# belinghy/SteppingStone

Measured on AMD Instinct MI355X. Metric: env-steps/sec (batched random-action rollout), higher is better.
Workload: dtype f32; 1 GPU; Walker3DStepperEnv-v0, 4096 envs per MI355X, curriculum 0 (flat terrain), on-device Philox U(-1,1) actions, auto-reset on; envs_total=4096, parallelism=env-shard x1, ranks=1, steps_per_launch=1000, prewarm_steps=256

## Files before the change

steppingstone_amd/csrc/ss_dynamics.hpp:

```cpp
#pragma once
#include "ss_math.hpp"
#include "ss_pair.hpp"

namespace ss {

constexpr float kH = 1.0f / 240.0f;
constexpr float kDt = 1.0f / 60.0f;
constexpr float kGrav = 9.8f;
constexpr float kPlankA = kStonePlankHalfLength, kPlankB = kStonePlankHalfWidth;
constexpr int kPgsIters = 5;
constexpr float kErp = 0.2f;
constexpr float kSlop = 0.001f;
constexpr float kVcorrMax = 2.0f;


constexpr int kWave = 64;
constexpr int kEnvsPerWave = 32;
constexpr int kLdsSlots = 40;
constexpr int kSlotsA = 20;
constexpr int kLdsC = 0;
constexpr int kLdsT = 18;
constexpr int kLdsHead = 36;
constexpr int kScalarBase = kSlotsA * kWave * 4;
constexpr int kRecWords = 9;
constexpr int kCholWords = 15 + 6;
constexpr int kHandJc = 0, kHandL0 = kHandJc + 8 * kRecWords, kHandLc = kHandL0 + kCholWords, kHandDet = 129, kHandAct = 146, kHandFloats = 158, kHandCs = kHandLc;
constexpr bool bias_offload(int helpers) { return helpers >= 3; }
constexpr bool spine_packed(int helpers) { return helpers >= 3; }
constexpr bool torques_paired(int helpers, bool kstep) { return helpers >= 3 && kstep; }
constexpr bool response_from_lds(int helpers, bool kstep) { return helpers >= 3 && kstep; }
constexpr int kHandBias = kHandJc;
static_assert(24 <= 3 * kRecWords, "biases fit the spine records' place");
constexpr int kHandRows = kHandJc + 3 * kRecWords;
constexpr int kHandRows3 = 160;
constexpr int kHandFloats3 = kHandRows3 + 40;
constexpr int kHandSlots3 = (kHandFloats3 + 3) / 4;
constexpr int hand_slots(int helpers) { return helpers >= 3 ? kHandSlots3 : (kHandFloats + 3) / 4; }
constexpr bool rows_offload(int helpers) { return helpers >= 3; }
constexpr int kHandSlots = (kHandFloats + 3) / 4;
static_assert(kLdsSlots + kHandSlots <= 80, "two helper-variant workgroups must fit the 160 KiB of a CU (16384 envs: 512 workgroups)");
static_assert(kHandRows + 40 <= kHandJc + 8 * kRecWords, "rows fit the leg records' place");
constexpr int kHandBase = kLdsSlots * kWave * 4;
constexpr int kFarWord0 = kHandLc;
constexpr int kFarBytes = (kHandBase + kFarWord0 * kWave) * 4;
static_assert(kFarBytes <= 65536, "every hand-off word beyond the offset field of the lane's own base goes through the far base");
constexpr bool hand_far(int idx) { return idx >= kFarWord0; }
constexpr int hand_far_offset(int idx) { return (idx - kFarWord0) * kWave * 4; }
constexpr int lds_bytes(int helpers) { return (kLdsSlots + hand_slots(helpers)) * kWave * 16; }
constexpr int hand_last_word(int helpers) { return hand_slots(helpers) * 4 - 1; }
static_assert(kHandFloats3 - 1 <= hand_last_word(3) && kHandFloats + 2 - 1 <= hand_last_word(1), "the words in use (one helper: + kHandOut2's two) are allocated");
static_assert(kFarBytes + (kWave - 1) * 4 + hand_far_offset(hand_last_word(1)) + 4 <= lds_bytes(1), "one helper: far base + largest word is inside the allocation");
static_assert(kFarBytes + (kWave - 1) * 4 + hand_far_offset(hand_last_word(3)) + 4 <= lds_bytes(3), "three helpers: far base + largest word is inside the allocation");
static_assert(hand_far_offset(kFarWord0) == 0 && hand_far_offset(hand_last_word(3)) < 65536 && hand_far_offset(hand_last_word(1)) < 65536,
              "every far offset fits the 16-bit offset field");
static_assert(hand_far_offset(1) - hand_far_offset(0) == 256 && hand_far_offset(hand_last_word(3)) / 256 <= 255,
              "far offsets are multiples of 256 B within ds_*2st64_b32's reach");
constexpr int NH = 12;
enum { S_ACT = 0, S_Q = 12, S_QD = 24, S_WLAM = 36, S_POS = 48, S_QUAT = 51, S_VW = 55, S_VV = 58, S_STP = 61, S_STN = 70,
       S_WKEY = 79, S_END = 80 };
static_assert(S_END <= (kLdsSlots - kSlotsA) * 4, "LDS scalar region overflow");
constexpr bool warm_in_lds(int helpers) { return helpers < 3; }
constexpr bool reset_pose_offload(int helpers, bool kstep) { return helpers >= 3 && kstep; }
constexpr int S_POSE = S_WLAM;
static_assert(!(reset_pose_offload(0, true) && warm_in_lds(0)) && !(reset_pose_offload(1, true) && warm_in_lds(1)) &&
              !(reset_pose_offload(2, true) && warm_in_lds(2)) && !(reset_pose_offload(3, true) && warm_in_lds(3)),
              "the reset pose lives where the warm-start impulses would: only a kernel that keeps those in registers has the words to spare");
static_assert(S_POSE + NH <= S_POS, "twelve words");
#ifndef SS_ARM_TAIL
#define SS_ARM_TAIL 1
#endif
#ifndef SS_BASE_TAIL
#define SS_BASE_TAIL 1
#endif
constexpr bool arm_tail_offload(int helpers, bool kstep) { return SS_ARM_TAIL != 0 && helpers >= 3 && kstep; }
constexpr bool base_tail_offload(int helpers, bool kstep) { return SS_BASE_TAIL != 0 && helpers >= 3 && kstep; }
constexpr bool limb_tail_offload(int helpers, bool kstep) { return arm_tail_offload(helpers, kstep) || base_tail_offload(helpers, kstep); }
constexpr int kHandArm = kHandRows3, kHandDv0 = kHandDet, kHandV0f = kHandDv0 + 6;
constexpr int kArmHelper = 1, kBaseHelper = 2;
static_assert(kHandArm + 4 * kRecWords <= kHandRows3 + 36, "the arm records fit the rows' directions");
static_assert(kHandV0f + 6 <= kHandDet + 13, "dv0 and v0f stay below the detection's flags word and the sole");
#ifndef SS_SPINE_TAU
#define SS_SPINE_TAU 1
#endif
constexpr bool spine_tau_offload(int helpers, bool kstep) { return SS_SPINE_TAU != 0 && helpers >= 3 && kstep; }
constexpr int kHandTau = kHandCs + 2 * NH, kTauHelper = 1;
static_assert(kHandTau >= kHandCs + 2 * NH && kHandTau + 6 <= kHandLc + 36 && kHandLc + 36 <= kHandDet,
              "the spine torques lie behind cos / sin, inside Lambda_own's 36 words, below the detection's");
static_assert(hand_far(kHandTau) && hand_far_offset(kHandTau + 5) <= hand_far_offset(hand_last_word(3)), "far words inside the three-helper allocation");
static_assert(bias_offload(3) && kTauHelper == 1, "the spine torques ride on helper 1's bias job");

constexpr int kHalf[NH] = {0, 1, 2, 3, 4, 5, 6, 7, 13, 14, 15, 16};
constexpr int left_twin(int jr) { return jr < 3 ? jr : (jr < 8 ? jr + 5 : jr + 4); }
constexpr bool mirror_flips(int j) { return kAxis[j] != 1; }
__host__ __device__ constexpr float mirror_sign(int j, float m) { return mirror_flips(j) ? m : 1.f; }
__host__ __device__ constexpr float action_lane_sign(int jr, float m) {
  return jr < 3 ? mirror_sign(jr, m) : (float)kPolicySign[jr];
}
__host__ __device__ constexpr float policy_true_sign(int jr, int side) {
  return jr < 3 ? 1.f : (float)kPolicySign[jr] * ((mirror_flips(jr) && side) ? -1.f : 1.f);
}
constexpr int first_child_half(int b) {
  int r = -1;
  for (int i = 0; i < NH; ++i)
    if (kParent[kHalf[i]] == b) r = kHalf[i] + 1;
  return r;
}

#define SS_MEMBAR() asm volatile("" ::: "memory")
#if defined(__HIP_DEVICE_COMPILE__)
#define SS_WAVE_SYNC() asm volatile("" ::: "memory")
#else
#define SS_WAVE_SYNC() ss_host_wave_sync()
#endif

#if defined(SS_PROFILE_PHASES) && defined(__HIP_DEVICE_COMPILE__)
struct Prof { uint32_t t[16]; uint32_t last; };
#define SS_PROF_DECL Prof& prof,
#define SS_PROF_ARG prof,
#define SS_PROF_RAW(i) do { uint32_t _n = __builtin_amdgcn_readfirstlane((uint32_t)__builtin_amdgcn_s_memtime()); \
    prof.t[i] = __builtin_amdgcn_readfirstlane(prof.t[i] + (_n - __builtin_amdgcn_readfirstlane(prof.last))); prof.last = _n; } while (0)
#ifdef SS_PROFILE_EPILOGUE
#define SS_PROF(i) SS_PROF_RAW(0)
#define SS_PROFE(i) SS_PROF_RAW(i)
#else
#define SS_PROF(i) SS_PROF_RAW(i)
#define SS_PROFE(i) ((void)0)
#endif
#else
#define SS_PROFE(i) ((void)0)
struct Prof { int unused; };
#define SS_PROF_DECL
#define SS_PROF_ARG
#define SS_PROF(i) ((void)0)
#endif

#if defined(SS_FUZZ_SCHED) && defined(__HIP_DEVICE_COMPILE__)
__device__ __forceinline__ void ss_fuzz(uint32_t site) {
  uint32_t h = (uint32_t)__builtin_amdgcn_s_memtime() ^ (site * 0x9E3779B9u);
  h *= 0x85EBCA6Bu; h ^= h >> 13; h *= 0xC2B2AE35u; h ^= h >> 16;
  h = __builtin_amdgcn_readfirstlane(h);
  const uint32_t n = ((h >> 8) & 3u) == 0u ? (h & 255u) : (h & 15u);
#pragma unroll 1
  for (uint32_t i = 0; i < n; ++i) __builtin_amdgcn_s_sleep(1);
}
#define SS_FUZZ(site) ss_fuzz(site)
#else
#define SS_FUZZ(site) ((void)0)
#endif

constexpr bool cs_offload(int helpers) { return helpers >= 3; }

struct Lds {
  float* base;
  int lane;
  SSD float2& q2(int item) const { return reinterpret_cast<float2*>(base)[item * kWave + lane]; }
  SSD float& s(int idx) const { return base[kScalarBase + idx * kWave + lane]; }
  SSD float& hs(int idx) const {
#if defined(__HIP_DEVICE_COMPILE__)
    if (hand_far(idx)) {
      int off = kFarBytes + lane * 4;
      asm("" : "+v"(off));
      return *reinterpret_cast<float*>(reinterpret_cast<char*>(base) + off + hand_far_offset(idx));
    }
#endif
    return base[kHandBase + idx * kWave + lane];
  }
};

struct Stones {
  float p[3][3], nrm[3][3], tilt[3][2];
};

struct FootReport {
  int contact;
  int on_target;
  float sole[3];
};

struct Warm {
  float lam[4][3];
  int key;
};
SSD void warm_clear(Warm& w) {
#pragma unroll
  for (int k = 0; k < 4; ++k) w.lam[k][0] = w.lam[k][1] = w.lam[k][2] = 0.f;
  w.key = 0;
}

template <class T>
struct JRecT {
  T cs, sn, Uw[3], Uv[3], Dinv, u;
};
using JRec = JRecT<float>;
using JRec2 = JRecT<ssf2>;
static_assert(sizeof(JRec2) == 2 * sizeof(JRec), "a pair record is two scalar records, nothing else");
struct JointCache {
  JRec r[NH];
  Chol6 L0;
};
constexpr int half_pos(int j) { return j <= 7 ? j : j - 5; }
SSD void put_rec_at(const Lds& L, int w, const JRec& r) {
  L.hs(w + 0) = r.cs; L.hs(w + 1) = r.sn; L.hs(w + 2) = r.Dinv;
#pragma unroll
  for (int m = 0; m < 3; ++m) { L.hs(w + 3 + m) = r.Uw[m]; L.hs(w + 6 + m) = r.Uv[m]; }
}
SSD void get_rec_at(const Lds& L, int w, JRec& r) {
  r.cs = L.hs(w + 0); r.sn = L.hs(w + 1); r.Dinv = L.hs(w + 2);
#pragma unroll
  for (int m = 0; m < 3; ++m) { r.Uw[m] = L.hs(w + 3 + m); r.Uv[m] = L.hs(w + 6 + m); }
}
SSD void put_rec(const Lds& L, int k, const JRec& r) { put_rec_at(L, kHandJc + k * kRecWords, r); }
SSD void get_rec(const Lds& L, int k, JRec& r) { get_rec_at(L, kHandJc + k * kRecWords, r); }
SSD void put_chol(const Lds& L, const Chol6& c) {
#pragma unroll
  for (int m = 0; m < 15; ++m) L.hs(kHandL0 + m) = c.l[m];
#pragma unroll
  for (int m = 0; m < 6; ++m) L.hs(kHandL0 + 15 + m) = c.di[m];
}
SSD void get_chol(const Lds& L, Chol6& c) {
#pragma unroll
  for (int i = 0; i < 15; ++i) c.l[i] = L.hs(kHandL0 + i);
#pragma unroll
  for (int i = 0; i < 6; ++i) c.di[i] = L.hs(kHandL0 + 15 + i);
}

SSD float xchg(float x) {
#if defined(__HIP_DEVICE_COMPILE__)
  return __builtin_bit_cast(float, __builtin_amdgcn_mov_dpp(__builtin_bit_cast(int, x), 0xB1, 0xF, 0xF, true));
#else
  return ss_host_xchg(x);
#endif
}
SSD uint32_t xchg_u32(uint32_t x) {
#if defined(__HIP_DEVICE_COMPILE__)
  return (uint32_t)__builtin_amdgcn_mov_dpp((int)x, 0xB1, 0xF, 0xF, true);
#else
  return __builtin_bit_cast(uint32_t, ss_host_xchg(__builtin_bit_cast(float, x)));
#endif
}
SSD int xchg_i(int x) {
#if defined(__HIP_DEVICE_COMPILE__)
  return __builtin_amdgcn_mov_dpp(x, 0xB1, 0xF, 0xF, true);
// ... 1324 lines not shown
```

steppingstone_amd/csrc/ss_kernels.hpp:

```cpp
#pragma once
#include <cstdlib>

#include "ss_dynamics.hpp"
#include "../../include/steppingstone.h"

namespace ss {

enum { F_POS = 0, F_QUAT = 3, F_VEL = 7, F_Q = 13, F_QD = 34, F_POT = 55, F_ZINIT = 56, F_EPRET = 57, F_NNDR = 58,
       F_STONE = 59, F_HEAD = 59 + 24, F_EPRET_LO = 59 + 30, NF = 59 + 30 + 1 };
enum { I_N = 0, I_COUNT = 1, I_ELAPSED = 2, I_RNG = 3, I_FLAGS = 4, I_PROV = 5, NI = 6 };
constexpr int kNumStones = 20;
constexpr int kNumSubsteps = 4;
constexpr float kDeg = 0.017453292519943295f;

struct Knobs {
  const float* prob;
  int per_env_prob;
  int curriculum;
  float power;
  int auto_reset;
};

struct Params {
  float* fstate;
// ... 483 lines not shown
    static_for<0, NH>([&](auto Kc) {
      constexpr int k = decltype(Kc)::value, jr = kHalf[k];
      constexpr int jl = left_twin(jr);
      const int gj = side ? jl : jr;
      if (jr >= 3 || side == 0) {
        Fo[(F_Q + gj) * np] = o.qt[k];
        Fo[(F_QD + gj) * np] = o.qdt[k];
        stage_obs_joint<Model, k>(stage, side, o.qt[k], o.qdt[k]);
      }
    });
    if (side == 0) {
      const float r2 = o.do_reset ? 0.f : o.roll, p2 = o.do_reset ? 0.f : o.pitch;
      const float cy = o.do_reset ? 1.f : o.cyaw, sy = o.do_reset ? 0.f : o.syaw;
      stage_obs_base(stage, o.pos, o.quat, o.v0, o.z_init, r2, p2, cy, sy, o.flags, &o.tgt[0][0], &o.tgt[0][3], &o.tgt[1][0], &o.tgt[1][3]);
      if (io.rew) io.rew[e] = o.r;
      if (io.done) io.done[e] = o.d ? 1 : 0;
      if (packed_layout) {
        stage[SS_OBS_DIM] = o.r;
        stage[SS_OBS_DIM + 1] = o.d ? 1.f : 0.f;
      }
      istage[0] = SS_F2U(o.inf.ep_ret); istage[1] = SS_F2U(o.inf.ep_len);
      istage[2] = (uint32_t)o.inf.bad_transition; istage[3] = (uint32_t)o.inf.steps_reached; istage[4] = (uint32_t)o.inf.update_terrain;
      istage[5] = SS_F2U(o.inf.ep_ret_lo);
#pragma unroll
      for (int i = 0; i < 3; ++i) Fo[(F_POS + i) * np] = o.pos[i];
#pragma unroll
      for (int i = 0; i < 4; ++i) Fo[(F_QUAT + i) * np] = o.quat[i];
#pragma unroll
      for (int i = 0; i < 3; ++i) { Fo[(F_VEL + i) * np] = o.v0.w[i]; Fo[(F_VEL + 3 + i) * np] = o.v0.v[i]; }
    }
  }
  {
    SS_WAVE_SYNC();
    const int env0 = (lane_global - lane) >> 1;
    const int nleft = P.n - env0;
    const int nvalid = nleft <= 0 ? 0 : (kEnvsPerWave < nleft ? kEnvsPerWave : nleft);
    auto copy_block = [&](float* dst, int nfl) {
      if ((reinterpret_cast<uintptr_t>(dst) & 15u) == 0) {
        const int n4 = nfl >> 2;
        float4* d4 = reinterpret_cast<float4*>(dst);
        const float4* s4 = reinterpret_cast<const float4*>(lds);
#pragma unroll 1
        for (int g = lane; g < n4; g += kWave) copy_out(&d4[g], s4[g]);
        for (int g = (n4 << 2) + lane; g < nfl; g += kWave) copy_out(&dst[g], lds[g]);
      } else {
#pragma unroll 1
        for (int g = lane; g < nfl; g += kWave) copy_out(&dst[g], lds[g]);
      }
    };
    if (io.obs) {
      float* og = io.obs + (size_t)env0 * SS_OBS_DIM;
      if (!packed_layout) {
        copy_block(og, nvalid * SS_OBS_DIM);
      } else {
#pragma unroll 1
        for (int g = lane; g < nvalid * SS_OBS_DIM; g += kWave) {
          const int el = g / SS_OBS_DIM, idx = g - el * SS_OBS_DIM;
          copy_out(&og[g], lds[el * kPackW + idx]);
        }
      }
    }
    if (io.packed) {
      float* pk = io.packed + (size_t)env0 * kPackW;
      if constexpr (ROLLOUT) pk += (long long)kstep * io.packed_step_stride;
      copy_block(pk, nvalid * kPackW);
    }
    if (io.info) {
      uint32_t* ig = reinterpret_cast<uint32_t*>(io.info + env0);
      const uint32_t* is = reinterpret_cast<const uint32_t*>(lds) + kInfoBase;
      for (int g = lane; g < nvalid * SS_INFO_WORDS; g += kWave) copy_out(&ig[g], is[g]);
    }
#if defined(__HIP_DEVICE_COMPILE__)
    if constexpr (!ROLLOUT) {
      if (io.peers) {
        constexpr int kPack = SS_OBS_DIM + 2;
        const PeerTable* T = io.peers;
        const int G = T->count;
        const size_t row0 = (size_t)T->rank * (size_t)T->n_local + (size_t)env0;
#pragma unroll 1
        for (int p = 0; p < G; ++p) copy_block(T->dst[p] + row0 * kPack, nvalid * kPack);
        __threadfence_system();
        if (lane == 0) {
          const uint32_t prev = atomicAdd(T->done_counter, 1u);
          if ((prev + 1u) % gridDim.x == 0u) {
            __threadfence_system();
            for (int p = 0; p < G; ++p)
              __hip_atomic_store(T->flag[p] + T->rank, io.flag_value, __ATOMIC_RELEASE, __HIP_MEMORY_SCOPE_SYSTEM);
          }
        }
      }
    }
#endif
  }
}

constexpr bool out_offload(int helpers, bool rollout) { return rollout && helpers >= 3; }
constexpr int kHandOut = kHandDet, kHandOut2 = kHandFloats;
static_assert(kHandOut2 + 2 <= kHandSlots * 4, "hand-off region");
constexpr int kHandCtr = kHandOut2 + 1;
static_assert(kHandCtr < kHandRows3, "below the rows' own words");
#if !defined(SS_HOST_HARNESS)
template <class Model, bool ROLLOUT>
__device__ __forceinline__ void emit_from_handoff(const Params& P, const StepIO& io, const Lds& L, int lane, int lane_global, int kstep,
                                                  float* lds) {
  const int e_raw = lane_global >> 1, side = lane_global & 1;
  const bool valid = e_raw < P.n;
  const int e = valid ? e_raw : P.n - 1;
  const float m = side ? -1.f : 1.f;
  StepOut o;
  get_base(L, m, o.pos, o.quat, o.v0);
  get_joints(L, m, o.qt, o.qdt);
  o.r = L.hs(kHandOut + 0);
  o.z_init = L.hs(kHandOut + 1);
  {
    const float w = L.hs(kHandOut + 2), w2 = xchg(w);
    o.inf.ep_ret = side ? w2 : w;
    o.inf.ep_ret_lo = side ? w : w2;
  }
  const int bits = __builtin_bit_cast(int, L.hs(kHandOut2 + 0));
  o.d = bits & 1;
  o.inf.bad_transition = (bits >> 1) & 1;
  o.inf.update_terrain = (bits >> 2) & 1;
  o.do_reset = (bits >> 3) & 1;
  o.flags = (bits >> 4) & 3;
  o.inf.steps_reached = (bits >> 8) & 31;
  o.inf.ep_len = (float)((bits >> 16) & 0xffff);
#pragma unroll
  for (int i = 0; i < 5; ++i) { o.tgt[0][i] = L.hs(kHandOut + 3 + i); o.tgt[1][i] = L.hs(kHandOut + 8 + i); }
  quat_roll_pitch_cs(o.quat, o.roll, o.pitch, o.cyaw, o.syaw);
  emit_outputs<Model, ROLLOUT>(P, io, o, e, side, valid, lane, lane_global, kstep, lds);
}
#endif

template <class Write>
SSD void random_actions_half(const Params& P, int e, int side, float m, uint32_t tt, Write&& write) {
  uint32_t ra[6][4];
#pragma unroll
  for (int b = 0; b < 6; ++b) philox4x32_10(6u * tt + b, 1u, P.env_offset + ((uint32_t)e & P.id_mask), 0u, P.seed_lo, P.seed_hi, ra[b]);
  static_for<0, NH>([&](auto Kc) {
    constexpr int k = decltype(Kc)::value, jr = kHalf[k];
    constexpr int jl = left_twin(jr);
    const float sg = action_lane_sign(jr, m);
    const uint32_t bits = side ? ra[jl / 4][jl % 4] : ra[jr / 4][jr % 4];
    write(k, sg * (2.f * u01(bits) - 1.f));
  });
}

struct StepScore {
  float pot_prev;
  bool d;
  int bad;
  float r, roll, pitch, cyaw, syaw;
};
SSD StepScore step_score(SS_PROF_DECL const float (&pos)[3], const float (&quat)[4], const Cache& c, const float (&target_old)[3],
                         const float (&sole)[2][3], float pot_prev, int advanced, int n, int elapsed, bool finite, float step_bonus,
                         float e_sum, float a2, int at_limit) {
  StepScore o;
  float pot = -planar_dist(target_old, pos) / kDt;
  SS_PROFE(4);
  float progress = pot - pot_prev;
  o.pot_prev = advanced ? -planar_dist(c.p[1], pos) / kDt : pot;
  float target_bonus = (n == kNumStones - 1 && planar_dist(c.p[1], pos) < 0.15f) ? 2.f : 0.f;
  float zs = fminf(sole[0][2], sole[1][2]);
  float tall_bonus = (pos[2] - zs > 0.7f) ? 2.f : -1.f;
  float zlow = fminf(fminf(c.p[0][2], c.p[1][2]), c.p[2][2]);
  bool d = (tall_bonus < 0.f) || (pos[2] < zlow + 0.3f) || !finite;
  bool timeout = elapsed >= SS_MAX_EPISODE_STEPS;
  o.bad = timeout ? 1 : 0;
  o.d = d || timeout;
  quat_roll_pitch_cs(quat, o.roll, o.pitch, o.cyaw, o.syaw);
  float posture = 0.f;
  if (!(o.pitch > -0.2f && o.pitch < 0.4f)) posture += fabsf(o.pitch);
  if (!(o.roll > -0.4f && o.roll < 0.4f)) posture += fabsf(o.roll);
  float energy = (4.5f / NJ) * (e_sum / NJ) + (0.225f / NJ) * (a2 / NJ);
  float r = progress + step_bonus + target_bonus + tall_bonus - energy - posture - 0.1f * (float)at_limit;
  if (!finite || !finite_bits(r)) r = 0.f;
  o.r = r;
  SS_PROFE(5);
  return o;
}
SSD void ep_return_add(float& ep_ret, float& ep_lo, float r) {
  const float s = ep_ret + r, bb = s - ep_ret;
  const float err = (ep_ret - (s - bb)) + (r - bb);
  const float lo = ep_lo + err;
  ep_ret = s + lo;
  ep_lo = lo - (ep_ret - s);
}

struct StepEnd {
  float pos[3], quat[4];
  SV v0;
  int flags, advanced;
  float hd[3][2];
  bool d;
  int bad;
  float r, roll, pitch, cyaw, syaw;
};
template <class Model, class Draw>
SSD void step_logic(SS_PROF_DECL const Lds& L, int side, float m, const FootReport& fr, Cache& c, float& pot_prev, float& nn_dr,
                    float& ep_ret, float& ep_lo, int& n, int& count, int& elapsed, uint32_t& ctr, bool store, Draw&& draw, StepEnd& o) {
  float (&pos)[3] = o.pos, (&quat)[4] = o.quat, (&hd)[3][2] = o.hd;
  SV& v0 = o.v0;
  get_base(L, m, pos, quat, v0);
  elapsed += 1;
  const float my_sole[3] = {fr.sole[0], m * fr.sole[1], fr.sole[2]};
  float ot_sole[3];
#pragma unroll
  for (int i = 0; i < 3; ++i) ot_sole[i] = xchg(my_sole[i]);
  const int ot_contact = xchg_i(fr.contact), ot_target = xchg_i(fr.on_target);
  float sole[2][3];
#pragma unroll
  for (int i = 0; i < 3; ++i) { sole[0][i] = side ? ot_sole[i] : my_sole[i]; sole[1][i] = side ? my_sole[i] : ot_sole[i]; }
  o.flags = side ? (ot_contact | (fr.contact << 1)) : (fr.contact | (ot_contact << 1));
  const int on_target = fr.on_target | ot_target;
  SS_PROFE(2);
  float accv = 0.f, e_sum = 0.f, a2 = 0.f;
  int at_limit = 0;
  static_for<0, NH>([&](auto Kc) {
    constexpr int k = decltype(Kc)::value, jr = kHalf[k];
    const float q = L.s(S_Q + k), qd = L.s(S_QD + k), a = L.s(S_ACT + k);
    const bool mine = (jr >= 3) || (side == 0);
    accv += q + qd;
    if (mine) {
      e_sum += fabsf(a * (0.1f * qd));
      a2 += a * a;
      if (at_joint_limit<Model, jr>(q)) at_limit += 1;
    }
  });
  accv += pos[0] + pos[1] + pos[2] + quat[0] + quat[1] + quat[2] + quat[3];
#pragma unroll
  for (int i = 0; i < 3; ++i) accv += v0.w[i] + v0.v[i];
  e_sum += xchg(e_sum);
  a2 += xchg(a2);
  at_limit += xchg_i(at_limit);
  const bool finite = finite_bits(accv) && (xchg_i(finite_bits(accv) ? 1 : 0) != 0);
  SS_PROFE(3);

  float target_old[3] = {c.p[1][0], c.p[1][1], c.p[1][2]};
  float step_bonus = 0.f;
  int advanced = 0;
#pragma unroll
  for (int sl = 0; sl < 3; ++sl) { hd[sl][0] = 1.f; hd[sl][1] = 0.f; }
  if (on_target != 0) {
    count += 1;
    if (count == 1) {
      float d0 = planar_dist(sole[0], target_old), d1 = planar_dist(sole[1], target_old);
      step_bonus = 50.f * expf(-fminf(d0, d1) / 0.25f);
    }
    if (count >= 2 && n < kNumStones - 1) {
      n += 1;
      count = 0;
      advanced = 1;
#pragma unroll
      for (int i = 0; i < 3; ++i) {
        c.p[0][i] = c.p[1][i]; c.nrm[0][i] = c.nrm[1][i];
        c.p[1][i] = c.p[2][i]; c.nrm[1][i] = c.nrm[2][i];
      }
      c.tilt[0][0] = c.tilt[1][0]; c.tilt[0][1] = c.tilt[1][1];
      c.tilt[1][0] = c.tilt[2][0]; c.tilt[1][1] = c.tilt[2][1];
      const float2 h1 = L.q2(kLdsHead + 1), h2 = L.q2(kLdsHead + 2);
      hd[0][0] = h1.x; hd[0][1] = m * h1.y;
      hd[1][0] = h2.x; hd[1][1] = m * h2.y;
      hd[2][0] = h2.x; hd[2][1] = m * h2.y;
      if (n + 1 <= kNumStones - 1) nn_dr = draw(ctr, n + 1, c.p[2], c.nrm[2], c.tilt[2], hd[2], store);
      L.q2(kLdsHead + 0) = h1;
      L.q2(kLdsHead + 1) = h2;
      L.q2(kLdsHead + 2) = make_float2(hd[2][0], m * hd[2][1]);
    }
  }
  o.advanced = advanced;
  const StepScore sc = step_score(SS_PROF_ARG pos, quat, c, target_old, sole, pot_prev, advanced, n, elapsed, finite, step_bonus, e_sum, a2, at_limit);
  pot_prev = sc.pot_prev;
  o.d = sc.d; o.bad = sc.bad; o.r = sc.r; o.roll = sc.roll; o.pitch = sc.pitch; o.cyaw = sc.cyaw; o.syaw = sc.syaw;
  ep_return_add(ep_ret, ep_lo, sc.r);
}

template <class Model, bool RANDOM_ACT, int HELPERS = 0, bool ROLLOUT = false>
SSD void step_env(const Params& P, const StepIO& io, int lane_global, int lane, float* lds) {
  static_assert(!ROLLOUT || RANDOM_ACT, "a multi-step launch draws its actions on the device");
  constexpr bool kOffload =
#if defined(__HIP_DEVICE_COMPILE__)
      out_offload(HELPERS, ROLLOUT);
#else
      false;
#endif
  constexpr bool kPose =
#if defined(__HIP_DEVICE_COMPILE__)
      reset_pose_offload(HELPERS, ROLLOUT);
#else
      false;
#endif
  static_assert(!kPose || kOffload, "the pose's helper and the counter's hand-off word are the output stage's kernel's");
  const int e_raw = lane_global >> 1, side = lane_global & 1;
  const bool valid = e_raw < P.n;
  int e = valid ? e_raw : P.n - 1;
  const size_t np = (size_t)P.npad;
  const float m = side ? -1.f : 1.f;
  const Lds L{lds, lane};
  float ain[NH];
  load_in<!RANDOM_ACT>(P, e, RANDOM_ACT ? nullptr : io.act + (size_t)e * NJ, side, m, L, ain);

  const int nsteps = ROLLOUT ? io.nsteps : 1;
#pragma unroll 1
  for (int kstep = 0; kstep < nsteps; ++kstep) {
  SS_FUZZ(0x60u);
  if constexpr (RANDOM_ACT) {
    bool drawn = false;
    if constexpr (ROLLOUT && HELPERS > 1) {
      if (kstep > 0) {
        float a[NH];
#pragma unroll
        for (int k = 0; k < NH; ++k) a[k] = L.hs(kHandAct + k);
#pragma unroll
        for (int k = 0; k < NH; ++k) L.s(S_ACT + k) = a[k];
        drawn = true;
      }
    }
    if (!drawn) random_actions_half(P, e, side, m, (uint32_t)io.t + (uint32_t)kstep, [&](int k, float a) { L.s(S_ACT + k) = a; });
  } else {
    put_actions(L, m, ain);
  }

  const float power = P.knobs->power;
  FootReport fr;
#if defined(SS_PROFILE_PHASES) && defined(__HIP_DEVICE_COMPILE__)
  Prof prof;
#pragma unroll
  for (int i = 0; i < 16; ++i) prof.t[i] = 0;
  prof.last = (uint32_t)__builtin_amdgcn_s_memtime();
#endif
  Warm wm;
  warm_clear(wm);
  if constexpr (warm_in_lds(HELPERS)) L.s(S_WKEY) = 0.f;
#pragma unroll 1
  for (int k = 0; k < kNumSubsteps; ++k) substep<Model, HELPERS, ROLLOUT>(SS_PROF_ARG power, fr, L, wm);
#if defined(__HIP_DEVICE_COMPILE__)
  if constexpr (limb_tail_offload(HELPERS, ROLLOUT)) {
    SS_PROF(11);
    __syncthreads();
    SS_FUZZ(0xCFu);
  }
#endif
  SS_FUZZ(0x61u);
  SS_PROF(12);
  SS_MEMBAR();
  SS_OPAQUE(e);
  const float* F = P.fstate + e;
  const Knobs K = *P.knobs;
  Cache c;
  load_cache(P, e, c);
  float pot_prev = F[F_POT * np], z_init = F[F_ZINIT * np];
  float ep_ret = F[F_EPRET * np], ep_lo = F[F_EPRET_LO * np], nn_dr = F[F_NNDR * np];
  int n = P.istate[e + I_N * np], count = P.istate[e + I_COUNT * np], elapsed = P.istate[e + I_ELAPSED * np];
  uint32_t ctr = (uint32_t)P.istate[e + I_RNG * np];
  const uint32_t ctr_in = ctr;
  SS_PROFE(1);

  float pos[3], quat[4];
  SV v0;
  get_base(L, m, pos, quat, v0);
  elapsed += 1;
  const float my_sole[3] = {fr.sole[0], m * fr.sole[1], fr.sole[2]};
  float ot_sole[3];
#pragma unroll
  for (int i = 0; i < 3; ++i) ot_sole[i] = xchg(my_sole[i]);
  const int ot_contact = xchg_i(fr.contact), ot_target = xchg_i(fr.on_target);
  float sole[2][3];
#pragma unroll
  for (int i = 0; i < 3; ++i) { sole[0][i] = side ? ot_sole[i] : my_sole[i]; sole[1][i] = side ? my_sole[i] : ot_sole[i]; }
  int flags = side ? (ot_contact | (fr.contact << 1)) : (fr.contact | (ot_contact << 1));
  const int on_target = fr.on_target | ot_target;
  SS_PROFE(2);
  float accv = 0.f, e_sum = 0.f, a2 = 0.f;
  int at_limit = 0;
  static_for<0, NH>([&](auto Kc) {
    constexpr int k = decltype(Kc)::value, jr = kHalf[k];
    const float q = L.s(S_Q + k), qd = L.s(S_QD + k), a = L.s(S_ACT + k);
    const bool mine = (jr >= 3) || (side == 0);
    accv += q + qd;
    if (mine) {
      e_sum += fabsf(a * (0.1f * qd));
      a2 += a * a;
      if (at_joint_limit<Model, jr>(q)) at_limit += 1;
    }
  });
  accv += pos[0] + pos[1] + pos[2] + quat[0] + quat[1] + quat[2] + quat[3];
#pragma unroll
  for (int i = 0; i < 3; ++i) accv += v0.w[i] + v0.v[i];
  e_sum += xchg(e_sum);
  a2 += xchg(a2);
  at_limit += xchg_i(at_limit);
  const bool finite = finite_bits(accv) && (xchg_i(finite_bits(accv) ? 1 : 0) != 0);
  SS_PROFE(3);

  float target_old[3] = {c.p[1][0], c.p[1][1], c.p[1][2]};
  float step_bonus = 0.f;
  int advanced = 0;
  float hd[3][2] = {{1.f, 0.f}, {1.f, 0.f}, {1.f, 0.f}};
  if (on_target != 0) {
    count += 1;
    if (count == 1) {
      float d0 = planar_dist(sole[0], target_old), d1 = planar_dist(sole[1], target_old);
      step_bonus = 50.f * expf(-fminf(d0, d1) / 0.25f);
    }
    if (count >= 2 && n < kNumStones - 1) {
      n += 1;
      count = 0;
      advanced = 1;
#pragma unroll
      for (int i = 0; i < 3; ++i) {
        c.p[0][i] = c.p[1][i]; c.nrm[0][i] = c.nrm[1][i];
        c.p[1][i] = c.p[2][i]; c.nrm[1][i] = c.nrm[2][i];
      }
      c.tilt[0][0] = c.tilt[1][0]; c.tilt[0][1] = c.tilt[1][1];
      c.tilt[1][0] = c.tilt[2][0]; c.tilt[1][1] = c.tilt[2][1];
      const float2 h1 = L.q2(kLdsHead + 1), h2 = L.q2(kLdsHead + 2);
      hd[0][0] = h1.x; hd[0][1] = m * h1.y;
      hd[1][0] = h2.x; hd[1][1] = m * h2.y;
      hd[2][0] = h2.x; hd[2][1] = m * h2.y;
      if (n + 1 <= kNumStones - 1) nn_dr = draw_stone(P, K, e, ctr, n + 1, c.p[2], c.nrm[2], c.tilt[2], hd[2], valid && side == 0);
      L.q2(kLdsHead + 0) = h1;
      L.q2(kLdsHead + 1) = h2;
      L.q2(kLdsHead + 2) = make_float2(hd[2][0], m * hd[2][1]);
    }
  }
  const StepScore sc = step_score(SS_PROF_ARG pos, quat, c, target_old, sole, pot_prev, advanced, n, elapsed, finite, step_bonus, e_sum, a2, at_limit);
  pot_prev = sc.pot_prev;
  const bool d = sc.d;
  const int bad = sc.bad;
  const float r = sc.r, roll = sc.roll, pitch = sc.pitch, cyaw = sc.cyaw, syaw = sc.syaw;
  ep_return_add(ep_ret, ep_lo, r);
  ss_info inf;
  inf.ep_ret = ep_ret;
  inf.ep_ret_lo = ep_lo;
  inf.ep_len = (float)elapsed;
  inf.bad_transition = bad;
  inf.steps_reached = n;
  inf.update_terrain = advanced;
  const bool do_reset = d && K.auto_reset;
  SS_PROFE(6);
  uint32_t rr[6][4];
  const bool pose_stale = kPose && do_reset && ctr != ctr_in;
  if (do_reset) {
    if (valid && side == 0) P.istate[e + I_PROV * np] = 0;
    flat_path(c);
#pragma unroll
    for (int sl = 0; sl < 3; ++sl) {
      hd[sl][0] = 1.f; hd[sl][1] = 0.f;
      L.q2(kLdsHead + sl) = make_float2(1.f, 0.f);
    }
    pos[0] = 0.f; pos[1] = 0.f; pos[2] = Model::stand_height + 0.01f;
    quat[0] = 1.f; quat[1] = quat[2] = quat[3] = 0.f;
#pragma unroll
    for (int i = 0; i < 3; ++i) { v0.w[i] = 0.f; v0.v[i] = 0.f; }
    if constexpr (kPose) {
      ctr += 6u;
    } else {
      uint32_t c3 = ctr + (side ? 3u : 0u), mine[3][4];
#pragma unroll
      for (int b = 0; b < 3; ++b) env_block(P, e, c3, mine[b]);
#pragma unroll
      for (int b = 0; b < 3; ++b)
#pragma unroll
        for (int i = 0; i < 4; ++i) {
          const uint32_t other = xchg_u32(mine[b][i]);
          rr[b][i] = side ? other : mine[b][i];
          rr[3 + b][i] = side ? mine[b][i] : other;
        }
      ctr += 6u;
    }
    z_init = pos[2];
    nn_dr = 0.75f;
    pot_prev = -planar_dist(c.p[1], pos) / kDt;
    n = 1; count = 0; elapsed = 0; flags = 0; ep_ret = 0.f; ep_lo = 0.f;
  }
  SS_PROFE(7);
  float qt[NH], qdt[NH];
  if constexpr (!kPose) {
    static_for<0, NH>([&](auto Kc) {
      constexpr int k = decltype(Kc)::value, jr = kHalf[k];
      constexpr int jl = left_twin(jr);
      const float sg = mirror_sign(jr, m);
      if (do_reset) {
        qt[k] = side ? reset_angle<Model, jl>(rr) : reset_angle<Model, jr>(rr);
        qdt[k] = 0.f;
      } else {
        qt[k] = sg * L.s(S_Q + k);
        qdt[k] = sg * L.s(S_QD + k);
      }
    });
  }
  SS_PROFE(8);
  SS_FUZZ(0x62u);
  if constexpr (ROLLOUT) {
    if (do_reset) {
      put_base(L, m, pos, quat, v0.w, v0.v);
      if constexpr (kPose) {
        float qp[NH];
#pragma unroll
        for (int k = 0; k < NH; ++k) qp[k] = L.s(S_POSE + k);
        const float zm = __builtin_bit_cast(float, side ? 0x80000000u : 0u);
        static_for<0, NH>([&](auto Kc) {
          constexpr int k = decltype(Kc)::value;
          L.s(S_Q + k) = qp[k];
          L.s(S_QD + k) = mirror_flips(kHalf[k]) ? zm : 0.f;
        });
      } else {
        put_joints(L, m, qt, qdt);
      }
    }
#if defined(__HIP_DEVICE_COMPILE__)
    if constexpr (kPose) {
      if (__any(pose_stale)) {
        if (pose_stale) reset_pose_half<Model>(P, e, side, m, ctr - 6u, [&](int k, float q) { L.s(S_Q + k) = q; });
      }
    }
#endif
    if (advanced || do_reset) put_stones(L, m, c);
  }
  if constexpr (kOffload) {
    L.hs(kHandOut + 0) = r;
    L.hs(kHandOut + 1) = z_init;
    L.hs(kHandOut + 2) = side ? inf.ep_ret_lo : inf.ep_ret;
    const int bits = (d ? 1 : 0) | (inf.bad_transition << 1) | (inf.update_terrain << 2) | ((do_reset ? 1 : 0) << 3) | (flags << 4) |
                     (inf.steps_reached << 8) | ((int)inf.ep_len << 16);
    L.hs(kHandOut2 + 0) = __builtin_bit_cast(float, bits);
    if constexpr (kPose) L.hs(kHandCtr) = __builtin_bit_cast(float, ctr);
#pragma unroll
    for (int i = 0; i < 3; ++i) { L.hs(kHandOut + 3 + i) = c.p[1][i]; L.hs(kHandOut + 8 + i) = c.p[2][i]; }
#pragma unroll
    for (int i = 0; i < 2; ++i) { L.hs(kHandOut + 6 + i) = c.tilt[1][i]; L.hs(kHandOut + 11 + i) = c.tilt[2][i]; }
  } else {
    StepOut o;
#pragma unroll
    for (int i = 0; i < 3; ++i) o.pos[i] = pos[i];
#pragma unroll
    for (int i = 0; i < 4; ++i) o.quat[i] = quat[i];
    o.v0 = v0;
#pragma unroll
    for (int k = 0; k < NH; ++k) { o.qt[k] = qt[k]; o.qdt[k] = qdt[k]; }
    o.r = r; o.z_init = z_init; o.roll = roll; o.pitch = pitch; o.cyaw = cyaw; o.syaw = syaw;
    o.d = d ? 1 : 0; o.flags = flags; o.do_reset = do_reset ? 1 : 0;
#pragma unroll
    for (int i = 0; i < 3; ++i) { o.tgt[0][i] = c.p[1][i]; o.tgt[1][i] = c.p[2][i]; }
#pragma unroll
    for (int i = 0; i < 2; ++i) { o.tgt[0][3 + i] = c.tilt[1][i]; o.tgt[1][3 + i] = c.tilt[2][i]; }
    o.inf = inf;
    emit_outputs<Model, ROLLOUT>(P, io, o, e, side, valid, lane, lane_global, kstep, lds);
  }
  if (valid && side == 0) {
  SS_PROFE(9);
    float* Fo = P.fstate + e;
    if (advanced || do_reset) {
      store_cache(P, e, c);
      store_headings(P, e, hd);
    }
    Fo[F_POT * np] = pot_prev;
    Fo[F_ZINIT * np] = z_init;
    Fo[F_EPRET * np] = ep_ret;
    Fo[F_EPRET_LO * np] = ep_lo;
    Fo[F_NNDR * np] = nn_dr;
    P.istate[e + I_N * np] = n;
    P.istate[e + I_COUNT * np] = count;
    P.istate[e + I_ELAPSED * np] = elapsed;
    P.istate[e + I_RNG * np] = (int)ctr;
    P.istate[e + I_FLAGS * np] = flags;
  }
  SS_MEMBAR();
#if defined(SS_PROFILE_PHASES) && defined(__HIP_DEVICE_COMPILE__)
  SS_PROFE(10);
  SS_PROF(13);
  if (lane == 0 && P.prof)
    for (int i = 0; i < 16; ++i) atomicAdd(P.prof + i, (unsigned long long)prof.t[i]);
#endif
  }
#if defined(__HIP_DEVICE_COMPILE__)
  if constexpr (out_offload(HELPERS, ROLLOUT)) __syncthreads();
#endif
}

#ifndef SS_HOST_HARNESS
template <class Model, bool RANDOM_ACT>
__global__ __launch_bounds__(kWave, 1) void step_kernel(Params P, StepIO io) {
  __shared__ float4 lds4[kLdsSlots * kWave];
  step_env<Model, RANDOM_ACT>(P, io, blockIdx.x * kWave + threadIdx.x, threadIdx.x, reinterpret_cast<float*>(lds4));
}
template <class Model, bool RANDOM_ACT, int HELPERS>
__global__ __launch_bounds__(kWave * (1 + HELPERS), 1) void step_kernel_helped(Params P, StepIO io) {
  __shared__ float4 lds4[(kLdsSlots + hand_slots(HELPERS)) * kWave];
  const int wave = __builtin_amdgcn_readfirstlane(threadIdx.x >> 6), lane = threadIdx.x & (kWave - 1);
  float* lds = reinterpret_cast<float*>(lds4);
  SS_FUZZ(0x70u + wave);
  if (wave == 0) {
    step_env<Model, RANDOM_ACT, HELPERS>(P, io, blockIdx.x * kWave + lane, lane, lds);
  } else {
    const Lds L{lds, lane};
#pragma unroll 1
    for (int k = 0; k < kNumSubsteps; ++k) helper_substep<Model, HELPERS, 6>(wave - 1, L, [](int) {});
  }
}
template <class Model>
__global__ __launch_bounds__(kWave, 1) void rollout_kernel(Params P, StepIO io) {
  __shared__ float4 lds4[kLdsSlots * kWave];
  step_env<Model, true, 0, true>(P, io, blockIdx.x * kWave + threadIdx.x, threadIdx.x, reinterpret_cast<float*>(lds4));
}
template <class Model, int HELPERS>
__global__ __launch_bounds__(kWave * (1 + HELPERS), 1) void rollout_kernel_helped(Params P, StepIO io) {
  __shared__ float4 lds4[(kLdsSlots + hand_slots(HELPERS)) * kWave];
  const int wave = __builtin_amdgcn_readfirstlane(threadIdx.x >> 6), lane = threadIdx.x & (kWave - 1);
  float* lds = reinterpret_cast<float*>(lds4);
  SS_FUZZ(0x70u + wave);
  if (wave == 0) {
    step_env<Model, true, HELPERS, true>(P, io, blockIdx.x * kWave + lane, lane, lds);
  } else {
    const Lds L{lds, lane};
    const int lane_global = blockIdx.x * kWave + lane, side = lane_global & 1;
    const int e = min(lane_global >> 1, P.n - 1);
    const float m = side ? -1.f : 1.f;
    constexpr int kPoseHelper = 0;
    const float power = spine_tau_offload(HELPERS, true) ? P.knobs->power : 0.f;
    uint32_t ctr_pose = 0u;
    if constexpr (reset_pose_offload(HELPERS, true))
      if (wave - 1 == kPoseHelper) ctr_pose = (uint32_t)P.istate[e + I_RNG * (size_t)P.npad];
#pragma unroll 1
    for (int kstep = 0; kstep < io.nsteps; ++kstep)
#pragma unroll 1
      for (int k = 0; k < kNumSubsteps; ++k) {
        helper_substep<Model, HELPERS, 4, spine_tau_offload(HELPERS, true)>(wave - 1, L, [&](int helper) {
          if (k != 0) return;
          SS_FUZZ(0x80u + helper);
          constexpr int kActHelper = 1, kEmitHelper = HELPERS - 1;
          if (HELPERS > 1 && helper == kActHelper && kstep + 1 < io.nsteps)
            random_actions_half(P, e, side, m, (uint32_t)io.t + (uint32_t)kstep + 1u, [&](int j, float a) { L.hs(kHandAct + j) = a; });
          if (out_offload(HELPERS, true) && helper == kEmitHelper && kstep > 0) emit_from_handoff<Model, true>(P, io, L, lane, lane_global, kstep - 1, lds);
        }, power);
        if constexpr (reset_pose_offload(HELPERS, true)) {
          if (k == 0 && wave - 1 == kPoseHelper) {
            SS_FUZZ(0xA0u);
            const uint32_t ctr_now = kstep == 0 ? ctr_pose : __builtin_bit_cast(uint32_t, L.hs(kHandCtr));
            if (kstep == 0 || __any(ctr_now != ctr_pose)) {
              ctr_pose = ctr_now;
              reset_pose_half<Model>(P, e, side, m, ctr_now, [&](int j, float q) { L.s(S_POSE + j) = q; });
            }
          }
        }
        if constexpr (limb_tail_offload(HELPERS, true)) {
          __syncthreads();
          SS_FUZZ(0xB0u + (wave - 1));
          if constexpr (arm_tail_offload(HELPERS, true))
            if (wave - 1 == kArmHelper) helper_arm_tail<Model>(L);
          if constexpr (base_tail_offload(HELPERS, true))
            if (wave - 1 == kBaseHelper) helper_base_tail(L);
          if (k == kNumSubsteps - 1) {
            __syncthreads();
            SS_FUZZ(0xC0u + (wave - 1));
          }
        }
      }
    if constexpr (out_offload(HELPERS, true)) {
      __syncthreads();
      SS_FUZZ(0x90u + wave);
      if (wave == 2) emit_from_handoff<Model, true>(P, io, L, lane, lane_global, io.nsteps - 1, lds);
    }
  }
}

template <class Model>
SSD void reset_env(const Params& P, int e, float* obs_row) {
  const size_t np = (size_t)P.npad;
  Dyn s;
  Cache c;
  uint32_t ctr = (uint32_t)P.istate[e + I_RNG * np];
  float pot, z_init, nn_dr;
  env_reset<Model>(P, e, s, c, ctr, pot, z_init, nn_dr);
  store_dyn(P, e, s);
  store_cache(P, e, c);
  const float straight[3][2] = {{1.f, 0.f}, {1.f, 0.f}, {1.f, 0.f}};
  store_headings(P, e, straight);
  P.fstate[e + F_POT * np] = pot;
  P.fstate[e + F_ZINIT * np] = z_init;
  P.fstate[e + F_EPRET * np] = 0.f;
  P.fstate[e + F_EPRET_LO * np] = 0.f;
  P.fstate[e + F_NNDR * np] = nn_dr;
  P.istate[e + I_N * np] = 1;
  P.istate[e + I_COUNT * np] = 0;
  P.istate[e + I_ELAPSED * np] = 0;
  P.istate[e + I_RNG * np] = (int)ctr;
  P.istate[e + I_FLAGS * np] = 0;
  if (obs_row) {
    float o[SS_OBS_DIM];
    write_obs<Model>(s, z_init, 0, c, o);
#pragma unroll
    for (int i = 0; i < SS_OBS_DIM; ++i) obs_row[i] = o[i];
  }
}

template <class Model>
__global__ __launch_bounds__(kWave) void reset_kernel(Params P, float* obs) {
  const int e = blockIdx.x * kWave + threadIdx.x;
  if (e >= P.n) return;
  reset_env<Model>(P, e, obs ? obs + (size_t)e * SS_OBS_DIM : nullptr);
}

template <class Model>
__global__ __launch_bounds__(kWave) void obs_kernel(Params P, float* obs) {
  const int e = blockIdx.x * kWave + threadIdx.x;
  if (e >= P.n) return;
  const size_t np = (size_t)P.npad;
  Dyn s;
  Cache c;
  load_dyn(P, e, s);
  load_cache(P, e, c);
  float o[SS_OBS_DIM];
  write_obs<Model>(s, P.fstate[e + F_ZINIT * np], P.istate[e + I_FLAGS * np], c, o);
#pragma unroll
  for (int i = 0; i < SS_OBS_DIM; ++i) obs[(size_t)e * SS_OBS_DIM + i] = o[i];
}
#endif

SSD void pack_env(const Params& P, int e, float* packed, size_t row) {
  const size_t np = (size_t)P.npad;
  float* o = packed + row * SS_STATE_DIM;
  for (int i = 0; i < 59; ++i) o[i] = P.fstate[e + (size_t)i * np];
  o[59] = (float)P.istate[e + I_N * np];
  o[60] = (float)P.istate[e + I_COUNT * np];
  o[61] = (float)P.istate[e + I_ELAPSED * np];
  uint32_t ctr = (uint32_t)P.istate[e + I_RNG * np];
  o[62] = (float)(ctr & 0xFFFFu);
  o[63] = (float)(ctr >> 16);
  o[64] = (float)P.istate[e + I_FLAGS * np];
  const int prov = P.istate[e + I_PROV * np];
  for (int i = 0; i < 120; ++i) {
    const int k = i / 6;
    o[65 + i] = k < prov ? P.terrain[e + (size_t)i * np] : (i % 6 == 0 ? 0.75f * (float)k : 0.f);
  }
  o[185] = P.fstate[e + (size_t)F_EPRET_LO * np];
}
SSD void pack_env(const Params& P, int e, float* packed) { pack_env(P, e, packed, (size_t)e); }
SSD void unpack_env(const Params& P, int e, const float* packed, size_t row) {
  const size_t np = (size_t)P.npad;
  const float* o = packed + row * SS_STATE_DIM;
  for (int i = 0; i < 59; ++i) P.fstate[e + (size_t)i * np] = o[i];
  int n = (int)o[59];
  P.istate[e + I_N * np] = n;
  P.istate[e + I_COUNT * np] = (int)o[60];
  P.istate[e + I_ELAPSED * np] = (int)o[61];
  P.istate[e + I_RNG * np] = (int)((uint32_t)o[62] | ((uint32_t)o[63] << 16));
  P.istate[e + I_FLAGS * np] = (int)o[64];
  for (int i = 0; i < 120; ++i) P.terrain[e + (size_t)i * np] = o[65 + i];
  P.istate[e + I_PROV * np] = kNumStones;
  P.fstate[e + (size_t)F_EPRET_LO * np] = o[185];
  Cache c;
  float hd[3][2];
  cache_from_terrain(P, e, n, c, hd);
  store_cache(P, e, c);
  store_headings(P, e, hd);
}
SSD void unpack_env(const Params& P, int e, const float* packed) { unpack_env(P, e, packed, (size_t)e); }

}
```

Measured before the change: 105.1 million env-steps/s.

## Offload step-epilogue roll/pitch computation to a helper wave

Adds an option for helper waves to compute parts of the step epilogue (joint-limit count, energy sums and finiteness, and roll/pitch from the base quaternion) after the last substep, handing results to the main wave through LDS words inside the existing allocation. By default only the posture (roll/pitch) offload is enabled, so the main wave skips quat_roll_pitch_cs and reads roll/pitch from LDS. This costs an extra __syncthreads barrier on both sides per step, which may outweigh the small amount of arithmetic removed.

```diff
diff --git a/steppingstone_amd/csrc/ss_dynamics.hpp b/steppingstone_amd/csrc/ss_dynamics.hpp
--- a/steppingstone_amd/csrc/ss_dynamics.hpp
+++ b/steppingstone_amd/csrc/ss_dynamics.hpp
@@ -88,6 +88,22 @@
               "the spine torques lie behind cos / sin, inside Lambda_own's 36 words, below the detection's");
 static_assert(hand_far(kHandTau) && hand_far_offset(kHandTau + 5) <= hand_far_offset(hand_last_word(3)), "far words inside the three-helper allocation");
 static_assert(bias_offload(3) && kTauHelper == 1, "the spine torques ride on helper 1's bias job");
+#ifndef SS_EPI_SUMS
+#define SS_EPI_SUMS 0
+#endif
+#ifndef SS_EPI_POSTURE
+#define SS_EPI_POSTURE 1
+#endif
+constexpr bool epi_sums_offload(int helpers, bool kstep) { return SS_EPI_SUMS != 0 && helpers >= 3 && kstep && limb_tail_offload(helpers, kstep); }
+constexpr bool epi_posture_offload(int helpers, bool kstep) { return SS_EPI_POSTURE != 0 && helpers >= 3 && kstep && limb_tail_offload(helpers, kstep); }
+constexpr bool epilogue_sums_offload(int helpers, bool kstep) { return epi_sums_offload(helpers, kstep) || epi_posture_offload(helpers, kstep); }
+constexpr int kHandEpi = kHandRows3;
+constexpr int kHandEpiWords = 6;
+constexpr int kEpiLimitHelper = 0, kEpiSumHelper = 1, kEpiPostureHelper = 2;
+static_assert(kHandEpi >= kHandRows3 && kHandEpi + kHandEpiWords <= kHandFloats3, "inside the rows' own words");
+static_assert(kHandEpi >= kHandFloats + 2 && kHandEpi > kHandAct + NH - 1 && kHandEpi > kHandDet + 16,
+              "above the output stage's words (kHandOut, kHandOut2, kHandCtr), the next step's actions and the detection's");
+static_assert(kHandEpi + kHandEpiWords - 1 <= hand_last_word(3) && lds_bytes(3) == 92160, "allocated; the kernel's LDS does not grow");
 
 constexpr int kHalf[NH] = {0, 1, 2, 3, 4, 5, 6, 7, 13, 14, 15, 16};
 constexpr int left_twin(int jr) { return jr < 3 ? jr : (jr < 8 ? jr + 5 : jr + 4); }
diff --git a/steppingstone_amd/csrc/ss_kernels.hpp b/steppingstone_amd/csrc/ss_kernels.hpp
--- a/steppingstone_amd/csrc/ss_kernels.hpp
+++ b/steppingstone_amd/csrc/ss_kernels.hpp
@@ -659,9 +659,10 @@
   int bad;
   float r, roll, pitch, cyaw, syaw;
 };
+template <bool POSTURE_GIVEN = false>
 SSD StepScore step_score(SS_PROF_DECL const float (&pos)[3], const float (&quat)[4], const Cache& c, const float (&target_old)[3],
                          const float (&sole)[2][3], float pot_prev, int advanced, int n, int elapsed, bool finite, float step_bonus,
-                         float e_sum, float a2, int at_limit) {
+                         float e_sum, float a2, int at_limit, float roll_given = 0.f, float pitch_given = 0.f) {
   StepScore o;
   float pot = -planar_dist(target_old, pos) / kDt;
   SS_PROFE(4);
@@ -675,7 +676,11 @@
   bool timeout = elapsed >= SS_MAX_EPISODE_STEPS;
   o.bad = timeout ? 1 : 0;
   o.d = d || timeout;
-  quat_roll_pitch_cs(quat, o.roll, o.pitch, o.cyaw, o.syaw);
+  if constexpr (POSTURE_GIVEN) {
+    o.roll = roll_given; o.pitch = pitch_given; o.cyaw = 0.f; o.syaw = 0.f;
+  } else {
+    quat_roll_pitch_cs(quat, o.roll, o.pitch, o.cyaw, o.syaw);
+  }
   float posture = 0.f;
   if (!(o.pitch > -0.2f && o.pitch < 0.4f)) posture += fabsf(o.pitch);
   if (!(o.roll > -0.4f && o.roll < 0.4f)) posture += fabsf(o.roll);
@@ -692,6 +697,54 @@
   const float lo = ep_lo + err;
   ep_ret = s + lo;
   ep_lo = lo - (ep_ret - s);
+}
+
+template <class Model>
+SSD void helper_epi_limits(const Lds& L, int side) {
+  int at_limit = 0;
+  static_for<0, NH>([&](auto Kc) {
+    constexpr int k = decltype(Kc)::value, jr = kHalf[k];
+    const float q = L.s(S_Q + k);
+    const bool mine = (jr >= 3) || (side == 0);
+    if (mine) {
+      if (at_joint_limit<Model, jr>(q)) at_limit += 1;
+    }
+  });
+  at_limit += xchg_i(at_limit);
+  L.hs(kHandEpi + 0) = __builtin_bit_cast(float, at_limit);
+}
+SSD void helper_epi_sums(const Lds& L, int side, float m) {
+  float pos[3], quat[4];
+  SV v0;
+  get_base(L, m, pos, quat, v0);
+  float accv = 0.f, e_sum = 0.f, a2 = 0.f;
+  static_for<0, NH>([&](auto Kc) {
+    constexpr int k = decltype(Kc)::value, jr = kHalf[k];
+    const float q = L.s(S_Q + k), qd = L.s(S_QD + k), a = L.s(S_ACT + k);
+    const bool mine = (jr >= 3) || (side == 0);
+    accv += q + qd;
+    if (mine) {
+      e_sum += fabsf(a * (0.1f * qd));
+      a2 += a * a;
+    }
+  });
+  accv += pos[0] + pos[1] + pos[2] + quat[0] + quat[1] + quat[2] + quat[3];
+#pragma unroll
+  for (int i = 0; i < 3; ++i) accv += v0.w[i] + v0.v[i];
+  e_sum += xchg(e_sum);
+  a2 += xchg(a2);
+  const bool finite = finite_bits(accv) && (xchg_i(finite_bits(accv) ? 1 : 0) != 0);
+  L.hs(kHandEpi + 1) = e_sum;
+  L.hs(kHandEpi + 2) = a2;
+  L.hs(kHandEpi + 3) = __builtin_bit_cast(float, finite ? 1 : 0);
+}
+SSD void helper_epi_posture(const Lds& L, float m) {
+  float pos[3], quat[4], roll, pitch, cyaw, syaw;
+  SV v0;
+  get_base(L, m, pos, quat, v0);
+  quat_roll_pitch_cs(quat, roll, pitch, cyaw, syaw);
+  L.hs(kHandEpi + 4) = roll;
+  L.hs(kHandEpi + 5) = pitch;
 }
 
 struct StepEnd {
@@ -798,6 +851,13 @@
       false;
 #endif
   static_assert(!kPose || kOffload, "the pose's helper and the counter's hand-off word are the output stage's kernel's");
+#if defined(__HIP_DEVICE_COMPILE__)
+  constexpr bool kEpiSums = epi_sums_offload(HELPERS, ROLLOUT), kEpiPosture = epi_posture_offload(HELPERS, ROLLOUT);
+#else
+  constexpr bool kEpiSums = false, kEpiPosture = false;
+#endif
+  constexpr bool kEpi = kEpiSums || kEpiPosture;
+  static_assert(!kEpi || kOffload, "roll / pitch as given: the output stage's helper forms its own, with cos / sin of the yaw");
   const int e_raw = lane_global >> 1, side = lane_global & 1;
   const bool valid = e_raw < P.n;
   int e = valid ? e_raw : P.n - 1;
@@ -880,6 +940,8 @@
   SS_PROFE(2);
   float accv = 0.f, e_sum = 0.f, a2 = 0.f;
   int at_limit = 0;
+  bool finite = true;
+  if constexpr (!kEpiSums) {
   static_for<0, NH>([&](auto Kc) {
     constexpr int k = decltype(Kc)::value, jr = kHalf[k];
     const float q = L.s(S_Q + k), qd = L.s(S_QD + k), a = L.s(S_ACT + k);
@@ -897,8 +959,9 @@
   e_sum += xchg(e_sum);
   a2 += xchg(a2);
   at_limit += xchg_i(at_limit);
-  const bool finite = finite_bits(accv) && (xchg_i(finite_bits(accv) ? 1 : 0) != 0);
+  finite = finite_bits(accv) && (xchg_i(finite_bits(accv) ? 1 : 0) != 0);
   SS_PROFE(3);
+  }
 
   float target_old[3] = {c.p[1][0], c.p[1][1], c.p[1][2]};
   float step_bonus = 0.f;
@@ -931,7 +994,27 @@
       L.q2(kLdsHead + 2) = make_float2(hd[2][0], m * hd[2][1]);
     }
   }
-  const StepScore sc = step_score(SS_PROF_ARG pos, quat, c, target_old, sole, pot_prev, advanced, n, elapsed, finite, step_bonus, e_sum, a2, at_limit);
+  float roll_given = 0.f, pitch_given = 0.f;
+#if defined(__HIP_DEVICE_COMPILE__)
+  if constexpr (kEpi) {
+    SS_PROFE(11);
+    __builtin_amdgcn_sched_barrier(0);
+    __syncthreads();
+    SS_FUZZ(0xEFu);
+    __builtin_amdgcn_sched_barrier(0);
+    SS_PROFE(12);
+    if constexpr (kEpiSums) {
+      at_limit = __builtin_bit_cast(int, L.hs(kHandEpi + 0));
+      e_sum = L.hs(kHandEpi + 1);
+      a2 = L.hs(kHandEpi + 2);
+      finite = __builtin_bit_cast(int, L.hs(kHandEpi + 3)) != 0;
+    }
+    if constexpr (kEpiPosture) { roll_given = L.hs(kHandEpi + 4); pitch_given = L.hs(kHandEpi + 5); }
+    SS_PROFE(3);
+  }
+#endif
+  const StepScore sc = step_score<kEpiPosture>(SS_PROF_ARG pos, quat, c, target_old, sole, pot_prev, advanced, n, elapsed, finite, step_bonus, e_sum, a2, at_limit,
+                                               roll_given, pitch_given);
   pot_prev = sc.pot_prev;
   const bool d = sc.d;
   const int bad = sc.bad;
@@ -1161,6 +1244,17 @@
           if (k == kNumSubsteps - 1) {
             __syncthreads();
             SS_FUZZ(0xC0u + (wave - 1));
+            if constexpr (epilogue_sums_offload(HELPERS, true)) {
+              if constexpr (epi_sums_offload(HELPERS, true)) {
+                if (wave - 1 == kEpiLimitHelper) helper_epi_limits<Model>(L, side);
+                if (wave - 1 == kEpiSumHelper) helper_epi_sums(L, side, m);
+              }
+              if constexpr (epi_posture_offload(HELPERS, true))
+                if (wave - 1 == kEpiPostureHelper) helper_epi_posture(L, m);
+              SS_FUZZ(0xD0u + (wave - 1));
+              __syncthreads();
+              SS_FUZZ(0xE0u + (wave - 1));
+            }
           }
         }
       }
```

Measured after the change: 105.7 million env-steps/s, median of 6. No clear change (+0.5%).
